# TheJacksonLaboratory/cnn_autoencoder

Hardware: AMD Instinct MI355X
Metric: tiles/sec, compress+decompress round trip of 1024x1024x3 histology tiles (higher is better)
Workload: dtype f32 (f16x3 split MFMA: 3 f16 MFMAs per product, fp32 accumulate)

## Files before the change

cnn_autoencoder_amd/_lib.py:

```python
from __future__ import annotations

import ctypes
import os
import subprocess
import threading

import torch

_HERE = os.path.dirname(os.path.abspath(__file__))
LIB_PATH = os.environ.get('CAE_LIB') or os.path.join(_HERE, 'libcae_hip.so')
_lock = threading.Lock()
_lib = None

c_void_p = ctypes.c_void_p
c_int = ctypes.c_int
c_size_t = ctypes.c_size_t
c_float = ctypes.c_float

SYMBOLS = {
    'cae_version': (c_int, []),
    'cae_last_error': (ctypes.c_char_p, []),
    'cae_free': (None, [c_void_p]),
    'cae_model_create': (c_int, [c_int, c_int, c_int, c_int, c_int, ctypes.POINTER(c_void_p)]),
    'cae_model_destroy': (None, [c_void_p]),
    'cae_model_set_layer': (c_int, [c_void_p, c_int, c_int, c_int, c_int, c_void_p, c_void_p, c_void_p, c_void_p]),
    'cae_model_set_layer_act': (c_int, [c_void_p, c_int, c_int, c_int, c_void_p, c_void_p]),
    'cae_model_set_precision': (c_int, [c_void_p, c_int]),
    'cae_last_range_ticket': (ctypes.c_int64, []),
    'cae_range_check': (c_int, [c_void_p, ctypes.c_int64, c_void_p]),
    'cae_thread_force_fp32': (None, [c_int]),
    'cae_model_effective_precision': (c_int, [c_void_p, c_void_p]),
    'cae_model_set_entropy': (c_int, [c_void_p, c_int, c_int, c_void_p, c_void_p, c_void_p, c_void_p]),
    'cae_analysis': (c_int, [c_void_p, c_void_p, c_int, c_int, c_int, c_int, c_void_p, c_void_p]),
    'cae_analysis_levels': (c_int, [c_void_p, c_void_p, c_int, c_int, c_int, c_int, c_void_p, c_void_p, c_void_p]),
    'cae_synthesis': (c_int, [c_void_p, c_void_p, c_int, c_int, c_int, c_void_p, c_int, c_void_p, c_void_p]),
    'cae_model_set_layer_stage': (c_int, [c_void_p, c_int, c_int, c_int, c_void_p, c_void_p, c_void_p, c_void_p, c_int,
                                           c_int, c_int]),
    'cae_model_set_color_layer': (c_int, [c_void_p, c_int, c_int, c_int, c_void_p, c_void_p]),
    'cae_synthesis_multiscale': (c_int, [c_void_p, c_void_p, c_int, c_int, c_int, c_void_p, c_int, c_void_p, c_void_p,
                                          c_void_p]),
    'cae_analysis_symbols': (c_int, [c_void_p, c_void_p, c_int, c_int, c_int, c_int, c_void_p, c_void_p]),
    'cae_synthesis_symbols': (c_int, [c_void_p, c_void_p, c_int, c_int, c_int, c_void_p, c_int, c_void_p]),
    'cae_synthesis_scale': (c_int, [c_void_p, c_void_p, c_int, c_int, c_int, c_int, c_void_p, c_int, c_void_p]),
    'cae_synthesis_symbols_scale': (c_int, [c_void_p, c_void_p, c_int, c_int, c_int, c_int, c_void_p, c_int, c_void_p]),
    'cae_gdn_forward': (c_int, [c_void_p, c_int, c_int, c_void_p, c_int, c_int, c_int, c_void_p, c_void_p]),
    'cae_quantize': (c_int, [c_void_p, c_void_p, c_int, c_int, c_void_p, c_void_p]),
    'cae_quantize_export': (c_int, [c_void_p, c_void_p, c_int, c_int, c_void_p, c_int, c_void_p]),
    'cae_copy_to_host': (c_int, [c_void_p, c_void_p, c_size_t]),
    'cae_dequantize': (c_int, [c_void_p, c_void_p, c_int, c_int, c_void_p, c_void_p]),
    'cae_model_set_density': (c_int, [c_void_p, c_int, c_int, c_void_p, c_void_p, c_void_p, c_void_p, c_float]),
    'cae_model_set_likelihood_form': (c_int, [c_void_p, c_int]),
    'cae_likelihood': (c_int, [c_void_p, c_void_p, c_int, c_int, c_void_p, c_void_p, c_void_p, c_void_p]),
    'cae_tile_ssim': (c_int, [c_void_p, c_void_p, c_int, c_int, c_int, c_int, c_void_p, c_void_p, c_size_t, c_void_p]),
    'cae_tile_delta_e': (c_int, [c_void_p, c_void_p, c_int, c_size_t, c_void_p, c_void_p, c_size_t, c_void_p]),
    'cae_u8hwc_to_planes': (c_int, [c_void_p, c_int, c_int, c_int, c_int, c_void_p, c_void_p]),
    'cae_avgpool2': (c_int, [c_void_p, c_int, c_int, c_int, c_void_p, c_void_p]),
    'cae_msssim_level': (c_int, [c_void_p, c_void_p, c_int, c_int, c_int, c_void_p, c_void_p, c_void_p, c_size_t, c_void_p]),
    'cae_tile_sse': (c_int, [c_void_p, c_void_p, c_int, c_size_t, c_void_p, c_void_p]),
    'cae_model_set_profiling': (c_int, [c_void_p, c_int]),
    'cae_model_get_profile': (c_int, [c_void_p, c_int, c_void_p, c_int, c_void_p, c_int]),
    'cae_t_packed_bytes': (c_size_t, [c_int, c_int, c_int]),
    'cae_t_pack_weights': (c_int, [c_void_p, c_int, c_int, c_int, c_int, c_void_p, c_void_p]),
    'cae_t_from_nchw': (c_int, [c_void_p, c_int, c_int, c_int, c_int, c_int, c_void_p, c_void_p, c_void_p]),
    'cae_t_to_nchw': (c_int, [c_void_p, c_int, c_int, c_int, c_int, c_int, c_void_p, c_void_p]),
    'cae_t_set_samples_per_block': (c_int, [c_int]),
# ... 116 lines not shown
        raise CaeError(f'libcae_hip error {rc}: {msg}')


def require_gpu() -> torch.device:
    if not torch.cuda.is_available():
        raise RuntimeError('cnn_autoencoder_amd: no HIP device is visible; the MI355X hot path has no CPU fallback')
    return torch.device('cuda', torch.cuda.current_device())


def stream_ptr() -> int:
    return torch.cuda.current_stream().cuda_stream


class Handle:

    def __init__(self, c_org: int, c_net: int, c_bn: int, level: int, ks: int):
        self._h = c_void_p()
        check(lib().cae_model_create(c_org, c_net, c_bn, level, ks, ctypes.byref(self._h)))

    @property
    def ptr(self):
        return self._h

    def close(self):
        if self._h:
            lib().cae_model_destroy(self._h)
            self._h = c_void_p()

    def __del__(self):
        try:
            self.close()
        except Exception:
            pass
```

cnn_autoencoder_amd/csrc/cae_api.hip:

```cpp
#include "cae_hip.h"
#include "cae_internal.hpp"
#include "cae_kernels.hpp"
#include "cae_kernels_f16.hpp"
#include "cae_launch.hpp"
#include "cae_pack.hpp"

#include <algorithm>
#include <cmath>
#include <cstdio>
#include <cstdlib>
#include <cstring>
#include <string>

namespace cae {

thread_local std::string g_last_error;
thread_local int64_t g_last_ticket = 0;
thread_local int g_force_fp32 = 0;

int fail(int code, const char *fmt, ...) {
    char buf[512];
    va_list ap;
    va_start(ap, fmt);
    vsnprintf(buf, sizeof buf, fmt, ap);
// ... 617 lines not shown
            if ((rc = launch_conv(m->ks, l.ct, l.gdn, l.cin, a, st))) return rc;
        }
        prof.end();
        if (!last && levels && levels[i]) {
            const size_t t2 = (size_t)n * l.cout * a.OH * a.OW;
            if (f16)
                hipLaunchKernelGGL(c8s_to_nchw_kernel<false>, dim3(ew_grid(t2)), dim3(256), 0, st, (const char *)a.out,
                                   levels[i], n, l.cout, a.OH, a.OW, l.ct * 4);
            else
                hipLaunchKernelGGL(c8_to_nchw_kernel, dim3(ew_grid(t2)), dim3(256), 0, st, (const float *)a.out,
                                   levels[i], n, l.cout, a.OH * a.OW, l.ct * 4);
            HIP_TRY(hipGetLastError());
        }
        cur = (const float *)a.out;
        cur_planes = l.ct * 4;
        ch = a.OH;
        cw = a.OW;
        cur_idx = out_idx;
    }
    return CAE_OK;
}

static int synthesis_impl(cae_model_t *mm, const float *latents, const int32_t *symbols, int n, int lh, int lw, void *out,
                          int fmt, float *const *bridges, float *const *colors, void *stream, int scale = 0);

int cae_synthesis(cae_model_t *mm, const float *latents, int n, int lh, int lw, void *out, int fmt,
                  float *const *bridges, void *stream) {
    if (!latents) return fail(CAE_ERR_ARG, "NULL argument");
    return synthesis_impl(mm, latents, nullptr, n, lh, lw, out, fmt, bridges, nullptr, stream);
}

int cae_synthesis_multiscale(cae_model_t *mm, const float *latents, int n, int lh, int lw, void *out, int fmt,
                             float *const *bridges, float *const *colors, void *stream) {
    if (!latents) return fail(CAE_ERR_ARG, "NULL argument");
    return synthesis_impl(mm, latents, nullptr, n, lh, lw, out, fmt, bridges, colors, stream);
}

int cae_synthesis_symbols(cae_model_t *mm, const int32_t *symbols, int n, int lh, int lw, void *out, int fmt,
                          void *stream) {
    if (!symbols) return fail(CAE_ERR_ARG, "NULL argument");
    return synthesis_impl(mm, nullptr, symbols, n, lh, lw, out, fmt, nullptr, nullptr, stream);
}

static int check_scale(cae_model_t *mm, int scale) {
    Model *m = reinterpret_cast<Model *>(mm);
    if (!m) return fail(CAE_ERR_ARG, "NULL argument");
    if (scale < 0 || scale >= m->L) return fail(CAE_ERR_ARG, "scale %d outside 0..%d", scale, m->L - 1);
    return CAE_OK;
}

int cae_synthesis_scale(cae_model_t *mm, const float *latents, int n, int lh, int lw, int scale, void *out, int fmt,
                        void *stream) {
    if (!latents) return fail(CAE_ERR_ARG, "NULL argument");
    CAE_TRY(check_scale(mm, scale));
    return synthesis_impl(mm, latents, nullptr, n, lh, lw, out, fmt, nullptr, nullptr, stream, scale);
}

int cae_synthesis_symbols_scale(cae_model_t *mm, const int32_t *symbols, int n, int lh, int lw, int scale, void *out,
                                int fmt, void *stream) {
    if (!symbols) return fail(CAE_ERR_ARG, "NULL argument");
    CAE_TRY(check_scale(mm, scale));
    return synthesis_impl(mm, nullptr, symbols, n, lh, lw, out, fmt, nullptr, nullptr, stream, scale);
}

static int synthesis_impl(cae_model_t *mm, const float *latents, const int32_t *symbols, int n, int lh, int lw, void *out,
                          int fmt, float *const *bridges, float *const *colors, void *stream, int scale) {
    Model *m = reinterpret_cast<Model *>(mm);
    if (!m || !out) return fail(CAE_ERR_ARG, "NULL argument");
    const int stop = m->L - 1 - scale, nrun = stop + 1;
    if (symbols && m->ent.channels == 0) return fail(CAE_ERR_ARG, "entropy model not set");
    if (n < 1 || lh < 1 || lw < 1) return fail(CAE_ERR_ARG, "bad latent batch %dx%dx%d", n, lh, lw);
    if (fmt != CAE_FMT_U8_HWC && fmt != CAE_FMT_F32_NCHW) return fail(CAE_ERR_ARG, "bad pixel format %d", fmt);
    for (auto &l : m->dec)
        if (!l.set) return fail(CAE_ERR_ARG, "synthesis layer not set");
    for (int i = 0; colors && i + 1 < m->L; ++i)
        if (colors[i] && ((lh << (i + 1)) <= m->ks / 2 || (lw << (i + 1)) <= m->ks / 2))
            return fail(CAE_ERR_ARG, "colour layer %d input %d x %d too small for reflect padding %d", i, lh << (i + 1),
                        lw << (i + 1), m->ks / 2);
    if (scale > 0) {
        const Layer &l = m->dec[stop];
        if (!l.color_wp) return fail(CAE_ERR_ARG, "colour layer %d not set", stop);
        if ((lh << nrun) <= m->ks / 2 || (lw << nrun) <= m->ks / 2)
            return fail(CAE_ERR_ARG, "colour layer %d input %d x %d too small for reflect padding %d", stop, lh << nrun,
                        lw << nrun, m->ks / 2);
    }
    hipStream_t st = (hipStream_t)stream;
    std::lock_guard<std::mutex> lk(m->mu);
    int rc;
    if ((rc = m->ensure_device()) || (rc = m->order_stream(stream))) return rc;
// ... 27 lines not shown
    if ((rc = m->ensure_ws(0, in_bytes))) return rc;
    if (maxact && ((rc = m->ensure_ws(1, maxact)) || (rc = m->ensure_ws(2, maxact)))) return rc;
    if (maxact && need_third_slot && (rc = m->ensure_ws(3, maxact))) return rc;

    ProfScope prof(m, CAE_SYNTHESIS, st);
    prof.begin();
    const size_t tot = (size_t)n * p0 * lh * lw;
    if (f16)
        hipLaunchKernelGGL(nchw_to_c8s_kernel<true>, dim3(ew_grid(tot)), dim3(256), 0, st, latents, (char *)m->ws[0].p, n,
                           m->c_bn, lh, lw, p0, flag, symbols, m->medians_dev.get<float>());
    else
        hipLaunchKernelGGL(nchw_to_c8_kernel, dim3(ew_grid(tot)), dim3(256), 0, st, latents, (float *)m->ws[0].p, n,
                           m->c_bn, lh * lw, p0, symbols, m->medians_dev.get<float>());
    HIP_TRY(hipGetLastError());
    prof.end();

    bool use_pmap = false;
    if (f16 && scale == 0 && m->L >= 2 && m->ks == 3 && getenv("CAE_NO_PMAP") == nullptr) {
        const Layer &lp = m->dec[m->L - 2], &ll = m->dec[m->L - 1];
        use_pmap = ll.wp_pmap16 && !ll.gdn && ll.stages.empty() && lp.stages.empty() && lp.ct <= 4 && lp.cout == ll.cin &&
                   !(bridges && bridges[m->L - 2]) && !(colors && colors[m->L - 2]);
    }
    if (use_pmap) maxact = std::max(maxact, (size_t)n * (lh << (m->L - 1)) * (lw << (m->L - 1)) * 128);
    if (use_pmap && ((rc = m->ensure_ws(1, maxact)) || (rc = m->ensure_ws(2, maxact)))) return rc;

    const float *cur = (const float *)m->ws[0].p;
    int cur_planes = p0, ch = lh, cw = lw;
    int cur_idx = 0;
    for (int i = 0; i < nrun; ++i) {
        const Layer &l = m->dec[i];
        const bool last = i == m->L - 1;
        if (use_pmap && last) {
            prof.begin();
            const int gtx = (cw + 15) / 16, gty = (ch + 15) / 16;
            hipLaunchKernelGGL(pmap_gather_kernel, dim3((unsigned)((size_t)n * gtx * gty)), dim3(256), 0, st, cur,
                               l.bias.get<float>(), out, n, ch, cw, l.cout, fmt == CAE_FMT_U8_HWC ? OUT_U8HWC : OUT_NCHW, gtx,
                               gty);
            HIP_TRY(hipGetLastError());
            prof.end();
            break;
        }
        if (!l.stages.empty() && (rc = run_stages(m, l, true, n, ch, cw, cur, cur_idx, cur_planes, st, f16, flag))) return rc;
        const int out_idx = pick_slot(cur_idx, cur_idx);
        LayerArgs a = layer_args(m, cur, cur_planes, last ? out : m->ws[out_idx].p, n, ch, cw, 2 * ch, 2 * cw, l.ct, l.cout,
                                 last ? (fmt == CAE_FMT_U8_HWC ? OUT_U8HWC : OUT_NCHW) : OUT_C8, l.act, flag);
        a.wp = l.wp.get<float>();
        a.bias = l.bias.get<float>();
        a.gp = l.gp.get<float>();
        a.beta = l.beta.get<float>();
        if (use_pmap && i == m->L - 2) {
            a.outfmt = OUT_PMAP;
            a.pm = m->dec[m->L - 1].wp_pmap16.p;
        }
        prof.begin();
        if (f16) {
            a.gp = l.gp16.get<float>();
            if (last && l.wp_edge16 && last_f16_fits(m->ks, l.cin)) {
                a.wp = l.wp_edge16.get<float>();
                if ((rc = launch_last_f16(m->ks, l.cin, a, st))) return rc;
            } else {
                if (l.act && l.ct > 4)
// ... 27 lines not shown
        }
        cur = (const float *)a.out;
        cur_planes = l.ct * 4;
        ch = a.OH;
        cw = a.OW;
        cur_idx = out_idx;
    }
    if (scale > 0) {
        const Layer &l = m->dec[stop];
        const int ofmt = fmt == CAE_FMT_U8_HWC ? OUT_U8HWC : OUT_NCHW;
        prof.begin();
        if (l.color_w4) {
            if ((rc = launch_color_small(m->ks, f16, cur, cur_planes, l.cout, l.color_w4.get<float>(),
                                         l.color_bias.get<float>(), n, ch, cw, l.color_cout, out, ofmt, flag, st)))
                return rc;
        } else {
            float *img = ofmt == OUT_NCHW ? (float *)out : (float *)m->ws[pick_slot(cur_idx, cur_idx)].p;
            if ((rc = launch_color(m, l, f16, cur, cur_planes, n, ch, cw, img, flag, st))) return rc;
            if (ofmt == OUT_U8HWC && (rc = launch_nchw_to_u8hwc(img, out, n, l.color_cout, (size_t)ch * cw, st))) return rc;
        }
        prof.end();
    }
    return CAE_OK;
}

int cae_gdn_forward(cae_model_t *mm, int track, int index, const float *x, int n, int h, int w, float *y, void *stream) {
    Model *m = reinterpret_cast<Model *>(mm);
    if (!m || !x || !y) return fail(CAE_ERR_ARG, "NULL argument");
    Layer *lp;
    CAE_TRY(layer_of(m, track, index, lp));
    if (n < 1 || h < 1 || w < 1) return fail(CAE_ERR_ARG, "bad tensor shape");
    hipStream_t st = (hipStream_t)stream;
    std::lock_guard<std::mutex> lk(m->mu);
    const Layer &l = *lp;
    if (!l.set || !l.gdn) return fail(CAE_ERR_ARG, "layer has no GDN");
    const int planes = l.ct * 4;
    int rc;
    if ((rc = m->ensure_device()) || (rc = m->order_stream(stream))) return rc;
    if ((rc = m->ensure_ws(0, (size_t)n * planes * h * w * 32))) return rc;
    const size_t tot = (size_t)n * planes * h * w;
    hipLaunchKernelGGL(nchw_to_c8_kernel, dim3(ew_grid(tot)), dim3(256), 0, st, x, (float *)m->ws[0].p, n, l.cout, h * w,
                       planes);
    HIP_TRY(hipGetLastError());
    LayerArgs a = layer_args(m, (const float *)m->ws[0].p, planes, y, n, h, w, h, w, l.ct, l.cout, OUT_NCHW, 0, nullptr);
    a.gp = l.gp.get<float>();
    a.beta = l.beta.get<float>();
// ... 284 lines not shown
```

cnn_autoencoder_amd/csrc/cae_kernels_f16.hpp:

```cpp
#pragma once
#include "cae_kernels.hpp"

namespace cae {

constexpr int F16_ISSUERS = 2;
#define ISSUER(w, NW, NI) ((w) < (NI) ? (w) : -1)

typedef _Float16 f16x8 __attribute__((ext_vector_type(8)));
typedef _Float16 f16x4 __attribute__((ext_vector_type(4)));


__device__ __forceinline__ void split_f16(float v, _Float16 &hi, _Float16 &lo) {
    hi = (_Float16)v;
    lo = (_Float16)(v - (float)hi);
}

typedef unsigned u32x2v __attribute__((ext_vector_type(2)));
__device__ __forceinline__ u32x2v split2_f16(float a, float b) {
    typedef float f32x2 __attribute__((ext_vector_type(2)));
    typedef _Float16 f16x2 __attribute__((ext_vector_type(2)));
    const f32x2 ab = {a, b};
    const unsigned hi = __builtin_bit_cast(unsigned, __builtin_convertvector(ab, f16x2));
    float l0, l1;
    asm("v_fma_mix_f32 %0, %1, -1.0, %2 op_sel_hi:[1,0,0]" : "=v"(l0) : "v"(hi), "v"(a));
// ... 727 lines not shown
            const f16x8 ah = *(const f16x8 *)(ab + ((jt * 2 + s) * 2 + 0) * 1024);
            const f16x8 al = *(const f16x8 *)(ab + ((jt * 2 + s) * 2 + 1) * 1024);
            pm = mfma3(ah, al, sh, sl, pm);
        }
    raise_if_over(mx, p.flag);
    __builtin_amdgcn_wave_barrier();
#pragma unroll
    for (int g = 0; g < 4; ++g) {
        const f32x4 v = {pm[4 * g], pm[4 * g + 1], pm[4 * g + 2], pm[4 * g + 3]};
        *(f32x4 *)(tbuf + m * 128 + (((2 * g + h) ^ (m & 7)) * 16)) = v;
    }
    __builtin_amdgcn_wave_barrier();
    const int half_w = p.OW >> 1;
    float *row = (float *)p.out + ((((size_t)n * p.OH + oy) * 2 + par) * half_w) * 32;
#pragma unroll
    for (int it = 0; it < 4; ++it) {
        const int px = (lane >> 3) + 8 * it, q = lane & 7;
        const f32x4 v = *(const f32x4 *)(tbuf + px * 128 + ((q ^ (px & 7)) * 16));
        if (row_valid && j0 + px < half_w) *(f32x4 *)(row + (size_t)(j0 + px) * 32 + 4 * q) = v;
    }
    __builtin_amdgcn_wave_barrier();
}

static __global__ void __launch_bounds__(256) pmap_gather_kernel(const float *pm, const float *bias, void *out, int N, int H,
                                                               int W, int cout, int fmt, int tiles_x, int tiles_y) {
    constexpr int T = 16, R = T + 1, PITCH = 36;
    __shared__ __attribute__((aligned(16))) float rec[R * R * PITCH];
    __shared__ __attribute__((aligned(4))) uint8_t orow[2 * T][2 * T * 3 + 4];
    int bid = blockIdx.x;
    const int tx = bid % tiles_x;
    bid /= tiles_x;
    const int ty = bid % tiles_y;
    const int n = bid / tiles_y;
    const int a0 = ty * T, b0 = tx * T;
    constexpr int NIT = (R * R * 8 + 255) / 256;
    f32x4 stage[NIT];
#pragma unroll
    for (int it = 0; it < NIT; ++it) {
        const int i = threadIdx.x + it * 256;
        const int q = i & 7, r = i >> 3;
        const int ra = r / R, rb = r - ra * R;
        const int a = a0 + ra, b = b0 + rb;
        stage[it] = f32x4{0.0f, 0.0f, 0.0f, 0.0f};
        if (i < R * R * 8 && a < H && b < W) stage[it] = *(const f32x4 *)(pm + pmap_record(n, H, W, a, b) + 4 * q);
    }
#pragma unroll
    for (int it = 0; it < NIT; ++it) {
        const int i = threadIdx.x + it * 256;
        if (i < R * R * 8) *(f32x4 *)(rec + (i >> 3) * PITCH + 4 * (i & 7)) = stage[it];
    }
    __syncthreads();
    const int la = threadIdx.x >> 4, lb = threadIdx.x & 15;
    const int a = a0 + la, b = b0 + lb;
    const float *p00 = rec + (la * R + lb) * PITCH, *p01 = p00 + PITCH, *p10 = p00 + R * PITCH, *p11 = p10 + PITCH;
    const int OH = 2 * H, OW = 2 * W;
    const bool u8 = fmt == OUT_U8HWC;
    typedef float f32x2 __attribute__((ext_vector_type(2)));
    const f32x4 s0 = *(const f32x4 *)(p00), s1 = *(const f32x4 *)(p00 + 4), s2 = *(const f32x4 *)(p00 + 8);
    const f32x4 l0 = *(const f32x4 *)(p01 + 12), u0 = *(const f32x4 *)(p10 + 20), d0 = *(const f32x4 *)(p11 + 28);
    const f32x2 l1 = *(const f32x2 *)(p01 + 16), u1 = *(const f32x2 *)(p10 + 24);
    const float self[12] = {s0[0], s0[1], s0[2], s0[3], s1[0], s1[1], s1[2], s1[3], s2[0], s2[1], s2[2], s2[3]};
    const float left[6] = {l0[0], l0[1], l0[2], l0[3], l1[0], l1[1]};
    const float up[6] = {u0[0], u0[1], u0[2], u0[3], u1[0], u1[1]};
    const float diag[3] = {d0[0], d0[1], d0[2]};
#pragma unroll
    for (int c = 0; c < 3; ++c) {
        if (c >= cout) break;
        const float bs = bias ? bias[c] : 0.0f;
        const float o00 = bs + self[c];
        const float o01 = bs + self[3 + c] + left[c];
        const float o10 = bs + self[6 + c] + up[c];
        const float o11 = bs + self[9 + c] + left[3 + c] + up[3 + c] + diag[c];
        if (u8) {
            orow[2 * la][(2 * lb) * cout + c] = clip_u8(o00 * 255.0f);
            orow[2 * la][(2 * lb + 1) * cout + c] = clip_u8(o01 * 255.0f);
            orow[2 * la + 1][(2 * lb) * cout + c] = clip_u8(o10 * 255.0f);
            orow[2 * la + 1][(2 * lb + 1) * cout + c] = clip_u8(o11 * 255.0f);
        } else if (a < H && b < W) {
            float *o = (float *)out + (((size_t)n * cout + c) * OH + 2 * a) * OW + 2 * b;
            o[0] = o00;
            o[1] = o01;
            o[OW] = o10;
            o[OW + 1] = o11;
        }
    }
    if (!u8) return;
    __syncthreads();
    const int row_bytes = 2 * T * cout;
    const int valid_rows = min(2 * T, OH - 2 * a0), valid_bytes = min(2 * T, OW - 2 * b0) * cout;
    uint8_t *obase = (uint8_t *)out + (((size_t)n * OH + 2 * a0) * OW + 2 * b0) * cout;
    const bool dwords = ((((size_t)OW * cout) & 3) == 0) && (((uintptr_t)obase & 3) == 0) && (row_bytes & 3) == 0 &&
                        valid_bytes == row_bytes;
    if (dwords) {
        const int per_row = row_bytes / 4;
        for (int i = threadIdx.x; i < valid_rows * per_row; i += 256) {
            const int r = i / per_row, q = i - r * per_row;
            *(uint32_t *)(obase + (size_t)r * OW * cout + 4 * q) = *(const uint32_t *)(&orow[r][4 * q]);
        }
    } else {
        for (int i = threadIdx.x; i < valid_rows * valid_bytes; i += 256) {
            const int r = i / valid_bytes, q = i - r * valid_bytes;
            obase[(size_t)r * OW * cout + q] = orow[r][q];
        }
    }
}

template <int KS, int CT, int NW, int PT, bool IGDN>
struct DeconvGeomF16 {
    static constexpr int P = KS / 2;
    static constexpr int DLO = -((P + 1) / 2), DHI = (KS - 1 - P) / 2;
    static constexpr int WH = 32 + DHI - DLO;
    static constexpr int ROWS = NW * PT;
    static constexpr int NSTRAY = WH - 32;
    static constexpr int AL_INSTR = 4 * ROWS * 32 / 64;
    static constexpr int AL_BYTES = AL_INSTR * 1024;
    static constexpr int STRAY_INSTR = (NSTRAY * 4 * ROWS + 63) / 64;
    static constexpr int HALO_INSTR = AL_INSTR + STRAY_INSTR;
    static_assert((4 * ROWS * 32) % 64 == 0 && 64 % (4 * ROWS) == 0, "halo image assumes 4, 8 or 16 input rows per block");
    static constexpr int W_INSTR = KS * CT * 2;
    static constexpr int W_BYTES = W_INSTR * 1024;
    static constexpr int G_BYTES = IGDN ? CT * 4096 : 0;
    static constexpr int CONV_STAGE = W_BYTES + HALO_INSTR * 1024;
    static constexpr int STAGE_BYTES = CONV_STAGE > G_BYTES ? CONV_STAGE : G_BYTES;
    static constexpr int NI = NW / F16_ISSUERS > 0 ? NW / F16_ISSUERS : 1;
    static constexpr int MAXP = (HALO_INSTR + NI - 1) / NI;
    static constexpr int AL_PER = AL_INSTR / NI, AL_STEP = NI * 64 / (ROWS * 32);
// ... 415 lines not shown
```

cnn_autoencoder_amd/csrc/cae_launch.hpp:

```cpp
#pragma once
#include <hip/hip_runtime.h>

#include <map>
#include <mutex>
#include <utility>

#include "cae_hip.h"
#include "cae_internal.hpp"

#define HIP_TRY(expr)                                                                             \
    do {                                                                                          \
        hipError_t e_ = (expr);                                                                   \
        if (e_ != hipSuccess) return ::cae::fail(CAE_ERR_HIP, "%s: %s", #expr, hipGetErrorString(e_));  \
    } while (0)

#define CAE_TRY(expr)                          \
    do {                                       \
        const int rc_ = (expr);                \
        if (rc_ != CAE_OK) return rc_;         \
    } while (0)

namespace cae {
inline std::mutex &launch_mutex() {
    static std::mutex mu;
// ... 36 lines not shown
    b.cci = cci;
    return b;
}

struct LayerArgs;
struct FirstArgs;
int launch_conv(int ks, int ct, bool gdn, int cin, const LayerArgs &a, hipStream_t st);
int launch_conv_s1(int ks, int ct, bool zeropad, bool gdn, int cin, const LayerArgs &a, hipStream_t st);
int launch_deconv(int ks, int ct, bool gdn, int cin, const LayerArgs &a, hipStream_t st);
int launch_gdn(int ct, bool inverse, const LayerArgs &a, hipStream_t st);
int launch_first(int ks, int ct, bool gdn, const LayerArgs &a, const FirstArgs &f, hipStream_t st);
int launch_last(int ks, int cin, const LayerArgs &a, hipStream_t st);
int launch_conv_f16(int ks, int ct, bool gdn, int cin, const LayerArgs &a, hipStream_t st);
int launch_deconv_f16(int ks, int ct, bool gdn, int cin, const LayerArgs &a, hipStream_t st);
int launch_conv_s1_f16(int ks, int ct, bool synthesis, bool gdn, int cin, const LayerArgs &a, hipStream_t st);
int launch_color_f16(int ks, int cin, const LayerArgs &a, hipStream_t st);
bool conv_f16_fits(int ks, int ct, bool gdn);
bool last_f16_fits(int ks, int cin);
int launch_color_small(int ks, bool split, const void *in, int in_planes, int cin, const float *w, const float *bias,
                       int n, int h, int w_px, int cout, void *out, int outfmt, int *flag, hipStream_t st);
int launch_nchw_to_u8hwc(const float *in, void *out, int n, int c, size_t hw, hipStream_t st);
int launch_first_f16(int ks, int ct, bool gdn, const LayerArgs &a, const FirstArgs &f, hipStream_t st);
int launch_last_f16(int ks, int cin, const LayerArgs &a, hipStream_t st);
int launch_gdn_f16(int ct, bool inverse, const LayerArgs &a, hipStream_t st);
}
```

cnn_autoencoder_amd/csrc/cae_launch_edge_f16.hip:

```cpp
#include <algorithm>

#include "cae_hip.h"
#include "cae_internal.hpp"
#include "cae_launch.hpp"
#include "cae_kernels_f16.hpp"
namespace cae {
template <int KS, int CT, bool GDN>
static int launch_first_f16_t(const LayerArgs &a, const FirstArgs &f, hipStream_t st) {
    using G = FirstGeomF16<KS, CT, GDN>;
    constexpr int LDS = G::LDS_BYTES;
    if constexpr (LDS > 160 * 1024) {
        return fail(CAE_ERR_UNSUPPORTED, "f16x3: first-layer operands exceed the LDS for this shape; use fp32");
    } else {
        auto kern_u8 = conv_first_f16_kernel<KS, CT, GDN, true>;
        auto kern_f32 = conv_first_f16_kernel<KS, CT, GDN, false>;
        int n_cu = 0;
        CAE_TRY(ensure_lds((const void *)kern_u8, LDS));
        CAE_TRY(ensure_lds((const void *)kern_f32, LDS));
        CAE_TRY(device_cus(n_cu));
        const LayerArgs b = with_launch_facts(a, a.OW, a.OH, G::TX, G::TY, (f.cin + 7) / 8);
        const size_t total = (size_t)b.N * b.tiles_x * b.tiles_y;
        if (total > 0x7fffffff) return fail(CAE_ERR_ARG, "batch too large");
        const unsigned grid = (unsigned)std::min<size_t>(total, (size_t)std::max(n_cu, 1));
        hipLaunchKernelGGL(f.in_is_u8 ? kern_u8 : kern_f32, dim3(grid), dim3(G::NW * 64), LDS, st, b, f);
// ... 54 lines not shown
static int launch_last_f16_t(int cin, const LayerArgs &a, hipStream_t st) {
    constexpr int NW = G::NW, DEPTH = G::DEPTH;
    const LayerArgs b = with_launch_facts(a, a.W, a.H, G::TXC, NW, (cin + 31) / 32);
    const int lds = G::lds_bytes(b.cci);
    if (lds > 160 * 1024) return fail(CAE_ERR_UNSUPPORTED, "last-layer weights do not fit the LDS");
    auto kern = deconv_last_f16_kernel<KS, NW, DEPTH>;
    int n_cu = 0;
    CAE_TRY(ensure_lds((const void *)kern, 160 * 1024));
    CAE_TRY(device_cus(n_cu));
    const size_t total = (size_t)b.N * b.tiles_x * b.tiles_y;
    if (total > 0x7fffffff) return fail(CAE_ERR_ARG, "batch too large");
    const unsigned grid = (unsigned)std::min<size_t>(total, (size_t)std::max(n_cu, 1));
    hipLaunchKernelGGL(kern, dim3(grid), dim3(NW * 64), lds, st, b);
    HIP_TRY(hipGetLastError());
    return CAE_OK;
}

int launch_last_f16(int ks, int cin, const LayerArgs &a, hipStream_t st) {
    if (ks == 3) return launch_last_f16_t<3, LastF16K3>(cin, a, st);
    if (ks == 5) return launch_last_f16_t<5, LastF16K5>(cin, a, st);
    return fail(CAE_ERR_UNSUPPORTED, "kernel_size %d not supported (3 or 5)", ks);
}

}
```

cnn_autoencoder_amd/modules.py:

```python
from __future__ import annotations

import ctypes
import math
from typing import List, Optional, Tuple

import numpy as np
import torch
import torch.nn as nn

from . import _lib
from .entropy import LowerBound

REPARAM_OFFSET = 2.0 ** -18


class RangeTicket:

    def __init__(self, track, handle, ticket: int, call):
        self._track, self._handle, self.ticket, self._call = track, handle, int(ticket), call

    def overflowed(self) -> bool:
        if self.ticket == 0:
            return False
        over = ctypes.c_int(0)
# ... 662 lines not shown
        if x.dim() != 4 or x.size(1) != self._dims[2]:
            raise ValueError(f'expected (B,{self._dims[2]},h,w), got {tuple(x.shape)}')
        hd = self._sync()
        x = x.detach().to(device=dev, dtype=torch.float32).contiguous()
        n, _, lh, lw = x.shape
        up = 2 ** (self._dims[3] - scale)

        def call():
            if fmt == _lib.FMT_U8_HWC:
                out = torch.empty((n, lh * up, lw * up, self._dims[0]), dtype=torch.uint8, device=dev)
            else:
                out = torch.empty((n, self._dims[0], lh * up, lw * up), dtype=torch.float32, device=dev)
            _lib.check(_lib.lib().cae_synthesis_scale(hd.ptr, x.data_ptr(), n, lh, lw, scale, out.data_ptr(), fmt,
                                                      _lib.stream_ptr()))
            return out
        return self._guarded(hd, call)

    def forward_scale(self, x: torch.Tensor, scale: int) -> torch.Tensor:
        return self._run_scale(x, scale, _lib.FMT_F32_NCHW)

    def forward_scale_u8(self, x: torch.Tensor, scale: int) -> torch.Tensor:
        return self._run_scale(x, scale, _lib.FMT_U8_HWC)

    def forward_symbols_u8(self, sym: torch.Tensor, eb, defer: bool = False, scale: int = 0):
        scale = self._check_scale(scale)
        dev = _lib.require_gpu()
        if sym.dim() != 4 or sym.size(1) != self._dims[2] or sym.dtype != torch.int32:
            raise ValueError(f'expected int32 (B,{self._dims[2]},h,w), got {sym.dtype} {tuple(sym.shape)}')
        if eb.channels != self._dims[2]:
            raise ValueError(f'entropy model has {eb.channels} channels, the latents {self._dims[2]}')
        sym = sym.to(dev).contiguous()
        hd = self._sync_entropy(eb)
        n, _, lh, lw = sym.shape
        L = self._dims[3]

        def call():
            up = 2 ** (L - scale)
            out = torch.empty((n, lh * up, lw * up, self._dims[0]), dtype=torch.uint8, device=dev)
            if scale == 0:
                _lib.check(_lib.lib().cae_synthesis_symbols(hd.ptr, sym.data_ptr(), n, lh, lw, out.data_ptr(),
                                                            _lib.FMT_U8_HWC, _lib.stream_ptr()))
            else:
                _lib.check(_lib.lib().cae_synthesis_symbols_scale(hd.ptr, sym.data_ptr(), n, lh, lw, scale,
                                                                  out.data_ptr(), _lib.FMT_U8_HWC, _lib.stream_ptr()))
            return out
        return self._guarded(hd, call, defer)
```

cnn_autoencoder_amd/slide.py:

```python
from __future__ import annotations

import math
from typing import Dict, List, Sequence, Tuple

import numpy as np
import torch

STATS_WIDTH = 3


def tile_range(rank: int, world: int, n_tiles: int) -> Tuple[int, int]:
    if not (0 <= rank < world) or n_tiles < 0:
        raise ValueError(f'bad partition request rank={rank} world={world} n_tiles={n_tiles}')
    base, rem = divmod(n_tiles, world)
    lo = rank * base + min(rank, rem)
    hi = lo + base + (1 if rank < rem else 0)
    return lo, hi


def tile_stats(nbytes: Sequence[int], sse: Sequence[float], n_samples: int) -> torch.Tensor:
    out = torch.empty((len(nbytes), STATS_WIDTH), dtype=torch.float64)
    out[:, 0] = torch.tensor(list(nbytes), dtype=torch.float64)
    out[:, 1] = torch.tensor(list(sse), dtype=torch.float64)
    out[:, 2] = float(n_samples)
# ... 281 lines not shown
                yield from emit(fut.result(), pl)
            while held:
                yield checked(*held.pop(0))
            while outgoing:
                yield outgoing.pop(0).result()

    def _pin(self, key, shape, dtype):
        buf = self._pinned.get(key)
        if buf is None or buf.shape != tuple(shape) or buf.dtype != dtype:
            buf = torch.empty(shape, dtype=dtype, pin_memory=True)
            self._pinned[key] = buf
        return buf

    @torch.no_grad()
    def run(self, batches: Sequence[torch.Tensor], keep_payloads: bool = False):
        import time
        from concurrent.futures import ThreadPoolExecutor
        from . import _lib
        dev = batches[0].device
        main = torch.cuda.current_stream(dev)
        copy_up = self._h2d_stream()
        K = len(batches)
        DEPTH = self.depth
        tm = dict(host_encode=0.0, host_decode=0.0, wait_host=0.0, d2h_copy=0.0)
        all_payloads, stats_parts = [], []
        device = self.coder == 'device'
        n0, h0, w0, _ = batches[0].shape
        lh0, lw0 = self.enc.latent_size(h0, w0)
        for j in range(0 if device else DEPTH + 2):
            self._pin(('a', j), (n0, self.eb.channels, lh0 * lw0), torch.int32)
        for j in range(0 if device else DEPTH + 2):
            self._pin(('d', j), (n0, self.eb.channels, lh0 * lw0), torch.int32)

        def stage_a(k):
            t = batches[k]
            sym, guard = self.enc.forward_u8_symbols(t, self.eb, defer=True)
            n, C = sym.size(0), sym.size(1)
            hw = sym.numel() // (n * C)
            pin = None if device else self._pin(('a', k % (DEPTH + 2)), (n, C, hw), torch.int32)
            ready = torch.cuda.Event(blocking=True)
            ready.record(main)
            return k, pin, ready, hw, sym, guard

        def host_pull(k, pin, ready, hw, sym, guard):
            ready.synchronize()
            if guard.overflowed():
# ... 23 lines not shown
            t0 = time.perf_counter()
            payloads = self._device_encode(k, sym)
            return k, payloads, hw, tuple(sym.shape), time.perf_counter() - t0

        def device_decode(enc_future):
            k, payloads, hw, shape, te = enc_future.result()
            t1 = time.perf_counter()
            sym = self._device_decode(k, payloads, hw)
            return payloads, sym, te, time.perf_counter() - t1

        def stage_d(k, payloads, back):
            t = batches[k]
            n, h, w, c = t.shape
            if device:
                sym = back
            else:
                with torch.cuda.stream(copy_up):
                    sym = back.to(dev, non_blocking=True)
                    up = torch.cuda.Event(blocking=True)
                    up.record(copy_up)
                main.wait_event(up)
            sym.record_stream(main)
            lh, lw = h // 2 ** self.level, w // 2 ** self.level
            rec, guard = self.dec.forward_symbols_u8(sym.reshape(n, self.eb.channels, lh, lw), self.eb, defer=True)
            sse = self.tile_sse(rec, t)
            got = torch.cuda.Event()
            got.record(main)
            sse_host = self._pin(('s', k % 4), (n,), torch.float64)
            with torch.cuda.stream(copy_up):
                copy_up.wait_event(got)
                sse_host.copy_(sse, non_blocking=True)
                landed = torch.cuda.Event(blocking=True)
                landed.record(copy_up)
            sse.record_stream(copy_up)
            nbytes = ([payloads.nbytes(i) + 16 for i in range(len(payloads))] if hasattr(payloads, 'nbytes')
                      else [len(p) + 16 for p in payloads])
            return (sse_host, landed), nbytes, h * w * c, guard, (k, payloads)

        pending = []

        def finalize(entry):
            (sse_pinned, landed), nbytes, samples, guard, (k, payloads) = entry
            landed.synchronize()
            sse_host = sse_pinned.tolist()
            if guard.overflowed():
                t = batches[k]
                rec = self._redo_synthesis(payloads, t.shape[1], t.shape[2], main)
                sse_host = self.tile_sse(rec, t).cpu().tolist()
            stats_parts.append(tile_stats(nbytes, sse_host, samples))

        workers = DEPTH if device else 1
        with ThreadPoolExecutor(max_workers=1) as pull_pool, ThreadPoolExecutor(max_workers=workers) as enc_pool, \
                ThreadPoolExecutor(max_workers=workers) as dec_pool:
            futs = {}

            def submit(k):
                if device:
# ... 25 lines not shown
```

include/cae_hip.h:

```cpp
#ifndef CAE_HIP_H
#define CAE_HIP_H

#include <stddef.h>
#include <stdint.h>

#ifdef __cplusplus
extern "C" {
#endif

typedef struct cae_model cae_model_t;

enum cae_status {
    CAE_OK = 0,
    CAE_ERR_ARG = -1,
    CAE_ERR_HIP = -2,
    CAE_ERR_NOMEM = -3,
    CAE_ERR_UNSUPPORTED = -4,
    CAE_ERR_CORRUPT = -5
};

enum cae_track { CAE_ANALYSIS = 0, CAE_SYNTHESIS = 1 };
enum cae_pixfmt {
    CAE_FMT_U8_HWC = 0,
    CAE_FMT_F32_NCHW = 1
// ... 25 lines not shown
                          const float *medians_host);

int cae_analysis(cae_model_t *m, const void *tiles_dev, int fmt, int n, int h, int w,
                 float *latents_dev, void *stream);

int cae_analysis_levels(cae_model_t *m, const void *tiles_dev, int fmt, int n, int h, int w, float *latents_dev,
                        float *const *levels_dev, void *stream);

int cae_synthesis(cae_model_t *m, const float *latents_dev, int n, int lh, int lw,
                  void *out_dev, int fmt, float *const *bridges_dev, void *stream);

int cae_model_set_layer_stage(cae_model_t *m, int track, int index, int stage, const float *w, const float *bias,
                              const float *beta, const float *gamma, int act, int add_residual, int post_act);

int cae_model_set_color_layer(cae_model_t *m, int index, int cin, int cout, const float *w, const float *bias);
int cae_synthesis_multiscale(cae_model_t *m, const float *latents_dev, int n, int lh, int lw, void *out_dev, int fmt,
                             float *const *bridges_dev, float *const *colors_dev, void *stream);

int cae_analysis_symbols(cae_model_t *m, const void *tiles_dev, int fmt, int n, int h, int w, int32_t *symbols_dev,
                         void *stream);
int cae_synthesis_symbols(cae_model_t *m, const int32_t *symbols_dev, int n, int lh, int lw, void *out_dev, int fmt,
                          void *stream);

int cae_synthesis_scale(cae_model_t *m, const float *latents_dev, int n, int lh, int lw, int scale, void *out_dev,
                        int fmt, void *stream);
int cae_synthesis_symbols_scale(cae_model_t *m, const int32_t *symbols_dev, int n, int lh, int lw, int scale,
                                void *out_dev, int fmt, void *stream);

int cae_gdn_forward(cae_model_t *m, int track, int index, const float *x_dev, int n, int h, int w,
                    float *y_dev, void *stream);

int cae_quantize(cae_model_t *m, const float *latents_dev, int n, int hw, int32_t *symbols_dev, void *stream);
int cae_dequantize(cae_model_t *m, const int32_t *symbols_dev, int n, int hw, float *latents_dev, void *stream);

int cae_quantize_export(cae_model_t *m, const float *latents_dev, int n, int hw, int32_t *symbols_pinned_host,
                        int max_blocks, void *stream);

int cae_model_set_density(cae_model_t *m, int channels, int n_filters, const int *filters,
                          const float *const *matrices, const float *const *biases,
                          const float *const *factors, float likelihood_bound);

int cae_model_set_likelihood_form(cae_model_t *m, int form);

int cae_likelihood(cae_model_t *m, const float *latents_dev, int n, int hw, float *y_hat_dev,
                   float *likelihood_dev, double *bits_dev, void *stream);

int cae_tile_ssim(const uint8_t *a_dev, const uint8_t *b_dev, int n, int h, int w, int c, double *ssim_dev,
                  double *workspace_dev, size_t workspace_elems, void *stream);

int cae_tile_delta_e(const uint8_t *a_dev, const uint8_t *b_dev, int n, size_t pixels, double *delta_dev,
// ... 138 lines not shown
```

Before: 4081.

## Fuse per-tile SSE into the final product-map gather kernel

Computes the reconstruction squared error against the reference tiles inside the last synthesis kernel, using udot4 on packed u8 dwords, a wave reduction and one 64-bit atomic per block. This replaces the separate tile_sse pass, which re-read the decoded tiles and the originals. Accumulators live in a device ring buffer that is periodically cleared by a memset, and the host copies integer SSE instead of float64. Reference bytes are prefetched into registers before the gather, which adds register pressure. The ring reuse depends on the slot count exceeding the pipeline depth.

Measured after the change: 4005. -1.9%, worse.

```diff
diff --git a/cnn_autoencoder_amd/_lib.py b/cnn_autoencoder_amd/_lib.py
--- a/cnn_autoencoder_amd/_lib.py
+++ b/cnn_autoencoder_amd/_lib.py
@@ -41,6 +41,9 @@
                                           c_void_p]),
     'cae_analysis_symbols': (c_int, [c_void_p, c_void_p, c_int, c_int, c_int, c_int, c_void_p, c_void_p]),
     'cae_synthesis_symbols': (c_int, [c_void_p, c_void_p, c_int, c_int, c_int, c_void_p, c_int, c_void_p]),
+    'cae_synthesis_symbols_sse': (c_int, [c_void_p, c_void_p, c_int, c_int, c_int, c_void_p, c_void_p, c_void_p, c_size_t,
+                                          ctypes.POINTER(c_int), c_void_p]),
+    'cae_pmap_gather_u8': (c_int, [c_void_p, c_void_p, c_int, c_int, c_int, c_int, c_void_p, c_void_p, c_void_p, c_void_p]),
     'cae_synthesis_scale': (c_int, [c_void_p, c_void_p, c_int, c_int, c_int, c_int, c_void_p, c_int, c_void_p]),
     'cae_synthesis_symbols_scale': (c_int, [c_void_p, c_void_p, c_int, c_int, c_int, c_int, c_void_p, c_int, c_void_p]),
     'cae_gdn_forward': (c_int, [c_void_p, c_int, c_int, c_void_p, c_int, c_int, c_int, c_void_p, c_void_p]),
@@ -203,6 +206,18 @@
     def ptr(self):
         return self._h
 
+    def sse_slot(self, n: int, slots: int, device):
+        S = max(2, int(slots))
+        ring = getattr(self, '_sse', None)
+        if ring is None or ring.shape != (2 * S, n) or ring.device != device:
+            ring = self._sse = torch.empty((2 * S, n), dtype=torch.int64, device=device)
+            self._sse_calls = 0
+        c = self._sse_calls
+        return ring[c % (2 * S)], (S * n if c % S == 0 else 0)
+
+    def sse_taken(self):
+        self._sse_calls += 1
+
     def close(self):
         if self._h:
             lib().cae_model_destroy(self._h)
diff --git a/cnn_autoencoder_amd/csrc/cae_api.hip b/cnn_autoencoder_amd/csrc/cae_api.hip
--- a/cnn_autoencoder_amd/csrc/cae_api.hip
+++ b/cnn_autoencoder_amd/csrc/cae_api.hip
@@ -663,7 +663,9 @@
 }
 
 static int synthesis_impl(cae_model_t *mm, const float *latents, const int32_t *symbols, int n, int lh, int lw, void *out,
-                          int fmt, float *const *bridges, float *const *colors, void *stream, int scale = 0);
+                          int fmt, float *const *bridges, float *const *colors, void *stream, int scale = 0,
+                          const uint8_t *ref = nullptr, unsigned long long *sse = nullptr, size_t sse_clear = 0,
+                          int *fused = nullptr);
 
 int cae_synthesis(cae_model_t *mm, const float *latents, int n, int lh, int lw, void *out, int fmt,
                   float *const *bridges, void *stream) {
@@ -704,8 +706,17 @@
     return synthesis_impl(mm, nullptr, symbols, n, lh, lw, out, fmt, nullptr, nullptr, stream, scale);
 }
 
+int cae_synthesis_symbols_sse(cae_model_t *mm, const int32_t *symbols, int n, int lh, int lw, void *out,
+                              const uint8_t *ref, unsigned long long *sse, size_t sse_clear, int *fused, void *stream) {
+    if (!symbols || !ref || !sse || !fused) return fail(CAE_ERR_ARG, "NULL argument");
+    *fused = 0;
+    return synthesis_impl(mm, nullptr, symbols, n, lh, lw, out, CAE_FMT_U8_HWC, nullptr, nullptr, stream, 0, ref, sse,
+                          sse_clear, fused);
+}
+
 static int synthesis_impl(cae_model_t *mm, const float *latents, const int32_t *symbols, int n, int lh, int lw, void *out,
-                          int fmt, float *const *bridges, float *const *colors, void *stream, int scale) {
+                          int fmt, float *const *bridges, float *const *colors, void *stream, int scale, const uint8_t *ref,
+                          unsigned long long *sse, size_t sse_clear, int *fused) {
     Model *m = reinterpret_cast<Model *>(mm);
     if (!m || !out) return fail(CAE_ERR_ARG, "NULL argument");
     const int stop = m->L - 1 - scale, nrun = stop + 1;
@@ -779,6 +790,9 @@
                    !(bridges && bridges[m->L - 2]) && !(colors && colors[m->L - 2]);
     }
     if (use_pmap) maxact = std::max(maxact, (size_t)n * (lh << (m->L - 1)) * (lw << (m->L - 1)) * 128);
+    const bool fuse_sse = use_pmap && ref && fmt == CAE_FMT_U8_HWC;
+    if (fuse_sse && sse_clear) HIP_TRY(hipMemsetAsync(sse, 0, sse_clear * sizeof(unsigned long long), st));
+    if (fused) *fused = fuse_sse ? 1 : 0;
     if (use_pmap && ((rc = m->ensure_ws(1, maxact)) || (rc = m->ensure_ws(2, maxact)))) return rc;
 
     const float *cur = (const float *)m->ws[0].p;
@@ -789,11 +803,10 @@
         const bool last = i == m->L - 1;
         if (use_pmap && last) {
             prof.begin();
-            const int gtx = (cw + 15) / 16, gty = (ch + 15) / 16;
-            hipLaunchKernelGGL(pmap_gather_kernel, dim3((unsigned)((size_t)n * gtx * gty)), dim3(256), 0, st, cur,
-                               l.bias.get<float>(), out, n, ch, cw, l.cout, fmt == CAE_FMT_U8_HWC ? OUT_U8HWC : OUT_NCHW, gtx,
-                               gty);
-            HIP_TRY(hipGetLastError());
+            if ((rc = launch_pmap_gather(cur, l.bias.get<float>(), out, n, ch, cw, l.cout,
+                                         fmt == CAE_FMT_U8_HWC ? OUT_U8HWC : OUT_NCHW, fuse_sse ? ref : nullptr,
+                                         fuse_sse ? sse : nullptr, st)))
+                return rc;
             prof.end();
             break;
         }
@@ -867,6 +880,13 @@
         prof.end();
     }
     return CAE_OK;
+}
+
+int cae_pmap_gather_u8(const float *pm, const float *bias, int n, int h, int w, int cout, uint8_t *out, const uint8_t *ref,
+                       unsigned long long *sse, void *stream) {
+    if (!pm || !out) return fail(CAE_ERR_ARG, "NULL argument");
+    if (n < 1 || h < 1 || w < 1) return fail(CAE_ERR_ARG, "bad map shape %dx%dx%d", n, h, w);
+    return launch_pmap_gather(pm, bias, out, n, h, w, cout, OUT_U8HWC, ref, sse, (hipStream_t)stream);
 }
 
 int cae_gdn_forward(cae_model_t *mm, int track, int index, const float *x, int n, int h, int w, float *y, void *stream) {
diff --git a/cnn_autoencoder_amd/csrc/cae_kernels_f16.hpp b/cnn_autoencoder_amd/csrc/cae_kernels_f16.hpp
--- a/cnn_autoencoder_amd/csrc/cae_kernels_f16.hpp
+++ b/cnn_autoencoder_amd/csrc/cae_kernels_f16.hpp
@@ -773,8 +773,10 @@
     __builtin_amdgcn_wave_barrier();
 }
 
+template <bool SSE>
 static __global__ void __launch_bounds__(256) pmap_gather_kernel(const float *pm, const float *bias, void *out, int N, int H,
-                                                               int W, int cout, int fmt, int tiles_x, int tiles_y) {
+                                                               int W, int cout, int fmt, int tiles_x, int tiles_y,
+                                                               const uint8_t *ref, unsigned long long *sse) {
     constexpr int T = 16, R = T + 1, PITCH = 36;
     __shared__ __attribute__((aligned(16))) float rec[R * R * PITCH];
     __shared__ __attribute__((aligned(4))) uint8_t orow[2 * T][2 * T * 3 + 4];
@@ -784,6 +786,30 @@
     const int ty = bid % tiles_y;
     const int n = bid / tiles_y;
     const int a0 = ty * T, b0 = tx * T;
+    const int OH = 2 * H, OW = 2 * W;
+    const int row_bytes = 2 * T * cout;
+    const int valid_rows = min(2 * T, OH - 2 * a0), valid_bytes = min(2 * T, OW - 2 * b0) * cout;
+    const size_t obase_off = (((size_t)n * OH + 2 * a0) * OW + 2 * b0) * cout;
+    uint8_t *obase = (uint8_t *)out + obase_off;
+    const bool dwords = ((((size_t)OW * cout) & 3) == 0) && (((uintptr_t)obase & 3) == 0) && (row_bytes & 3) == 0 &&
+                        valid_bytes == row_bytes;
+    const int per_row = row_bytes / 4;
+    constexpr int ND = (2 * T * (2 * T * 3 / 4) + 255) / 256;
+    const uint8_t *rbase = nullptr;
+    bool ref_dwords = false;
+    uint32_t rpre[ND] = {};
+    if constexpr (SSE) {
+        rbase = ref + obase_off;
+        ref_dwords = dwords && ((uintptr_t)rbase & 3) == 0;
+        if (ref_dwords) {
+#pragma unroll
+            for (int j = 0; j < ND; ++j) {
+                const int i = threadIdx.x + 256 * j;
+                const int r = i / per_row, q = i - r * per_row;
+                if (i < valid_rows * per_row) rpre[j] = *(const uint32_t *)(rbase + (size_t)r * OW * cout + 4 * q);
+            }
+        }
+    }
     constexpr int NIT = (R * R * 8 + 255) / 256;
     f32x4 stage[NIT];
 #pragma unroll
@@ -804,7 +830,6 @@
     const int la = threadIdx.x >> 4, lb = threadIdx.x & 15;
     const int a = a0 + la, b = b0 + lb;
     const float *p00 = rec + (la * R + lb) * PITCH, *p01 = p00 + PITCH, *p10 = p00 + R * PITCH, *p11 = p10 + PITCH;
-    const int OH = 2 * H, OW = 2 * W;
     const bool u8 = fmt == OUT_U8HWC;
     typedef float f32x2 __attribute__((ext_vector_type(2)));
     const f32x4 s0 = *(const f32x4 *)(p00), s1 = *(const f32x4 *)(p00 + 4), s2 = *(const f32x4 *)(p00 + 8);
@@ -837,22 +862,49 @@
     }
     if (!u8) return;
     __syncthreads();
-    const int row_bytes = 2 * T * cout;
-    const int valid_rows = min(2 * T, OH - 2 * a0), valid_bytes = min(2 * T, OW - 2 * b0) * cout;
-    uint8_t *obase = (uint8_t *)out + (((size_t)n * OH + 2 * a0) * OW + 2 * b0) * cout;
-    const bool dwords = ((((size_t)OW * cout) & 3) == 0) && (((uintptr_t)obase & 3) == 0) && (row_bytes & 3) == 0 &&
-                        valid_bytes == row_bytes;
+    unsigned err = 0;
     if (dwords) {
-        const int per_row = row_bytes / 4;
-        for (int i = threadIdx.x; i < valid_rows * per_row; i += 256) {
-            const int r = i / per_row, q = i - r * per_row;
-            *(uint32_t *)(obase + (size_t)r * OW * cout + 4 * q) = *(const uint32_t *)(&orow[r][4 * q]);
+        if constexpr (SSE) {
+#pragma unroll
+            for (int j = 0; j < ND; ++j) {
+                const int i = threadIdx.x + 256 * j;
+                if (i < valid_rows * per_row) {
+                    const int r = i / per_row, q = i - r * per_row;
+                    const uint32_t v = *(const uint32_t *)(&orow[r][4 * q]);
+                    *(uint32_t *)(obase + (size_t)r * OW * cout + 4 * q) = v;
+                    uint32_t w = rpre[j];
+                    if (!ref_dwords) {
+                        const uint8_t *rp = rbase + (size_t)r * OW * cout + 4 * q;
+                        w = (uint32_t)rp[0] | ((uint32_t)rp[1] << 8) | ((uint32_t)rp[2] << 16) | ((uint32_t)rp[3] << 24);
+                    }
+                    err += __builtin_amdgcn_udot4(v, v, __builtin_amdgcn_udot4(w, w, 0u, false), false) -
+                           2u * __builtin_amdgcn_udot4(v, w, 0u, false);
+                }
+            }
+        } else {
+            for (int i = threadIdx.x; i < valid_rows * per_row; i += 256) {
+                const int r = i / per_row, q = i - r * per_row;
+                *(uint32_t *)(obase + (size_t)r * OW * cout + 4 * q) = *(const uint32_t *)(&orow[r][4 * q]);
+            }
         }
     } else {
         for (int i = threadIdx.x; i < valid_rows * valid_bytes; i += 256) {
             const int r = i / valid_bytes, q = i - r * valid_bytes;
             obase[(size_t)r * OW * cout + q] = orow[r][q];
-        }
+            if constexpr (SSE) {
+                const int d = (int)orow[r][q] - (int)rbase[(size_t)r * OW * cout + q];
+                err += (unsigned)(d * d);
+            }
+        }
+    }
+    if constexpr (SSE) {
+        __shared__ unsigned wave_err[4];
+#pragma unroll
+        for (int off = 32; off > 0; off >>= 1) err += __shfl_down(err, off, 64);
+        if ((threadIdx.x & 63) == 0) wave_err[threadIdx.x >> 6] = err;
+        __syncthreads();
+        if (threadIdx.x == 0)
+            atomicAdd(sse + n, (unsigned long long)(wave_err[0] + wave_err[1] + wave_err[2] + wave_err[3]));
     }
 }
 
diff --git a/cnn_autoencoder_amd/csrc/cae_launch.hpp b/cnn_autoencoder_amd/csrc/cae_launch.hpp
--- a/cnn_autoencoder_amd/csrc/cae_launch.hpp
+++ b/cnn_autoencoder_amd/csrc/cae_launch.hpp
@@ -82,5 +82,7 @@
 int launch_nchw_to_u8hwc(const float *in, void *out, int n, int c, size_t hw, hipStream_t st);
 int launch_first_f16(int ks, int ct, bool gdn, const LayerArgs &a, const FirstArgs &f, hipStream_t st);
 int launch_last_f16(int ks, int cin, const LayerArgs &a, hipStream_t st);
+int launch_pmap_gather(const float *pm, const float *bias, void *out, int n, int h, int w, int cout, int outfmt,
+                       const uint8_t *ref, unsigned long long *sse, hipStream_t st);
 int launch_gdn_f16(int ct, bool inverse, const LayerArgs &a, hipStream_t st);
 }
diff --git a/cnn_autoencoder_amd/csrc/cae_launch_edge_f16.hip b/cnn_autoencoder_amd/csrc/cae_launch_edge_f16.hip
--- a/cnn_autoencoder_amd/csrc/cae_launch_edge_f16.hip
+++ b/cnn_autoencoder_amd/csrc/cae_launch_edge_f16.hip
@@ -100,4 +100,18 @@
     return fail(CAE_ERR_UNSUPPORTED, "kernel_size %d not supported (3 or 5)", ks);
 }
 
+int launch_pmap_gather(const float *pm, const float *bias, void *out, int n, int h, int w, int cout, int outfmt,
+                       const uint8_t *ref, unsigned long long *sse, hipStream_t st) {
+    if (cout < 1 || cout > 3) return fail(CAE_ERR_UNSUPPORTED, "product-map gather writes at most 3 channels, not %d", cout);
+    if ((ref != nullptr) != (sse != nullptr) || (ref && outfmt != OUT_U8HWC))
+        return fail(CAE_ERR_ARG, "the fused tile error needs uint8 output, the reference tiles and the accumulators");
+    const int gtx = (w + 15) / 16, gty = (h + 15) / 16;
+    const size_t total = (size_t)n * gtx * gty;
+    if (total > 0x7fffffff) return fail(CAE_ERR_ARG, "batch too large");
+    hipLaunchKernelGGL(ref ? pmap_gather_kernel<true> : pmap_gather_kernel<false>, dim3((unsigned)total), dim3(256), 0, st, pm,
+                       bias, out, n, h, w, cout, outfmt, gtx, gty, ref, sse);
+    HIP_TRY(hipGetLastError());
+    return CAE_OK;
 }
+
+}
diff --git a/cnn_autoencoder_amd/modules.py b/cnn_autoencoder_amd/modules.py
--- a/cnn_autoencoder_amd/modules.py
+++ b/cnn_autoencoder_amd/modules.py
@@ -708,7 +708,9 @@
     def forward_scale_u8(self, x: torch.Tensor, scale: int) -> torch.Tensor:
         return self._run_scale(x, scale, _lib.FMT_U8_HWC)
 
-    def forward_symbols_u8(self, sym: torch.Tensor, eb, defer: bool = False, scale: int = 0):
+    sse_ring_slots = 8
+
+    def forward_symbols_u8(self, sym: torch.Tensor, eb, defer: bool = False, scale: int = 0, ref: torch.Tensor = None):
         scale = self._check_scale(scale)
         dev = _lib.require_gpu()
         if sym.dim() != 4 or sym.size(1) != self._dims[2] or sym.dtype != torch.int32:
@@ -719,10 +721,26 @@
         hd = self._sync_entropy(eb)
         n, _, lh, lw = sym.shape
         L = self._dims[3]
+        if ref is not None:
+            want = (n, lh * 2 ** L, lw * 2 ** L, self._dims[0])
+            if scale != 0:
+                raise ValueError('ref: the tile error is taken at full resolution only (scale 0)')
+            if tuple(ref.shape) != want or ref.dtype != torch.uint8:
+                raise ValueError(f'expected uint8 reference tiles {want}, got {ref.dtype} {tuple(ref.shape)}')
+            ref = ref.to(dev).contiguous()
 
         def call():
             up = 2 ** (L - scale)
             out = torch.empty((n, lh * up, lw * up, self._dims[0]), dtype=torch.uint8, device=dev)
+            if ref is not None:
+                acc, clear = hd.sse_slot(n, self.sse_ring_slots, dev)
+                fused = ctypes.c_int(0)
+                _lib.check(_lib.lib().cae_synthesis_symbols_sse(hd.ptr, sym.data_ptr(), n, lh, lw, out.data_ptr(),
+                                                                ref.data_ptr(), acc.data_ptr(), clear, ctypes.byref(fused),
+                                                                _lib.stream_ptr()))
+                if fused.value:
+                    hd.sse_taken()
+                return out, (acc if fused.value else None)
             if scale == 0:
                 _lib.check(_lib.lib().cae_synthesis_symbols(hd.ptr, sym.data_ptr(), n, lh, lw, out.data_ptr(),
                                                             _lib.FMT_U8_HWC, _lib.stream_ptr()))
@@ -730,4 +748,8 @@
                 _lib.check(_lib.lib().cae_synthesis_symbols_scale(hd.ptr, sym.data_ptr(), n, lh, lw, scale,
                                                                   out.data_ptr(), _lib.FMT_U8_HWC, _lib.stream_ptr()))
             return out
-        return self._guarded(hd, call, defer)
+        res = self._guarded(hd, call, defer)
+        if ref is not None and defer:
+            (out, sse), guard = res
+            return out, guard, sse
+        return res
diff --git a/cnn_autoencoder_amd/slide.py b/cnn_autoencoder_amd/slide.py
--- a/cnn_autoencoder_amd/slide.py
+++ b/cnn_autoencoder_amd/slide.py
@@ -327,6 +327,7 @@
         copy_up = self._h2d_stream()
         K = len(batches)
         DEPTH = self.depth
+        self.dec.sse_ring_slots = max(self.dec.sse_ring_slots, DEPTH + 2)
         tm = dict(host_encode=0.0, host_decode=0.0, wait_host=0.0, d2h_copy=0.0)
         all_payloads, stats_parts = [], []
         device = self.coder == 'device'
@@ -396,17 +397,19 @@
                 main.wait_event(up)
             sym.record_stream(main)
             lh, lw = h // 2 ** self.level, w // 2 ** self.level
-            rec, guard = self.dec.forward_symbols_u8(sym.reshape(n, self.eb.channels, lh, lw), self.eb, defer=True)
-            sse = self.tile_sse(rec, t)
+            rec, guard, acc = self.dec.forward_symbols_u8(sym.reshape(n, self.eb.channels, lh, lw), self.eb, defer=True,
+                                                          ref=t)
+            sse = acc if acc is not None else self.tile_sse(rec, t)
             got = torch.cuda.Event()
             got.record(main)
-            sse_host = self._pin(('s', k % 4), (n,), torch.float64)
+            sse_host = self._pin(('s', k % 4), (n,), sse.dtype)
             with torch.cuda.stream(copy_up):
                 copy_up.wait_event(got)
                 sse_host.copy_(sse, non_blocking=True)
                 landed = torch.cuda.Event(blocking=True)
                 landed.record(copy_up)
-            sse.record_stream(copy_up)
+            if acc is None:
+                sse.record_stream(copy_up)
             nbytes = ([payloads.nbytes(i) + 16 for i in range(len(payloads))] if hasattr(payloads, 'nbytes')
                       else [len(p) + 16 for p in payloads])
             return (sse_host, landed), nbytes, h * w * c, guard, (k, payloads)
diff --git a/include/cae_hip.h b/include/cae_hip.h
--- a/include/cae_hip.h
+++ b/include/cae_hip.h
@@ -71,10 +71,17 @@
 int cae_synthesis_symbols(cae_model_t *m, const int32_t *symbols_dev, int n, int lh, int lw, void *out_dev, int fmt,
                           void *stream);
 
+int cae_synthesis_symbols_sse(cae_model_t *m, const int32_t *symbols_dev, int n, int lh, int lw, void *out_dev,
+                              const uint8_t *ref_dev, unsigned long long *sse_dev, size_t sse_clear, int *fused,
+                              void *stream);
+
 int cae_synthesis_scale(cae_model_t *m, const float *latents_dev, int n, int lh, int lw, int scale, void *out_dev,
                         int fmt, void *stream);
 int cae_synthesis_symbols_scale(cae_model_t *m, const int32_t *symbols_dev, int n, int lh, int lw, int scale,
                                 void *out_dev, int fmt, void *stream);
+
+int cae_pmap_gather_u8(const float *pm_dev, const float *bias_dev, int n, int h, int w, int cout, uint8_t *out_dev,
+                       const uint8_t *ref_dev, unsigned long long *sse_dev, void *stream);
 
 int cae_gdn_forward(cae_model_t *m, int track, int index, const float *x_dev, int n, int h, int w,
                     float *y_dev, void *stream);
```
